# NTT123/vietTTS

Hardware: NVIDIA H100
Metric: audio_samples_per_sec (higher is better)
Workload: dtype f32 (bf16x3 split products on wgmma tensor cores, fp32 accumulate/storage)

## Files before the change

### viettts_b200/csrc/tc_conv.cu

```cuda
#include <cuda_bf16.h>

#include <algorithm>

#include "tc_common.cuh"
#include "vtts_internal.cuh"

namespace {

using namespace tcx;

constexpr int NCWG = 2;
constexpr int NCONS = NCWG * 128;
constexpr int PROD_WARP = NCONS / 32;
constexpr int NCONV = 96;
constexpr int NTHREADS = NCONS + 32 + NCONV;
constexpr int NA = 4;
constexpr int HALO = 64;
constexpr int PAIR_OVERLAP = 16;
constexpr int NQ = 2;
constexpr int NREADERS = (NCONS + NCONV) / 32;

constexpr int SUB_CG = 4;
constexpr int SUB_HALO = 1;
constexpr int SUB_RS = NCWG * 64 + SUB_HALO;
constexpr int SUB_CSB = SUB_RS * 64 + 32;
constexpr int SUB_STAGE = SUB_CG * SUB_CSB;
static_assert(SUB_RS * 4 % 32 == 4 && SUB_CSB / 4 % 32 == 24, "bank-conflict-free converter stores");

template <int N, int MW, int PAIRF, bool STAGED = false, bool SUB = false>
struct TcCfg {
  static constexpr int R = 64 * MW * NCWG;
  static constexpr int R_OUT = R - PAIR_OVERLAP;
  static constexpr int RA = R + HALO;
  static constexpr int A_STAGE = RA * 64;
  static constexpr int NAS = SUB ? (N == 64 ? 4 : 2) : NA;
  static constexpr int A_BYTES = SUB ? NAS * SUB_STAGE : NA * A_STAGE;
  static constexpr int W_STAGE = N * 64;
  static constexpr int NW = N == 256 ? 4 : 8;
  static constexpr int NCH2 = PAIRF ? N / 16 : 0;
  static constexpr int EPI_NC = N < 128 ? N : 128;
  static constexpr int EPI_LD = EPI_NC + 8;
  static constexpr int EPI_WG = 64 * EPI_LD + N;
  static constexpr int EPI_STAGE = STAGED ? NCWG * EPI_WG * 4 : 0;
  static constexpr int SMEM_BYTES =
      A_BYTES + NW * W_STAGE + NCH2 * A_STAGE + EPI_STAGE + (2 * NA + 2 * NW + 2 * NQ) * 8 + NQ * 4 + 1024;
  static_assert(SMEM_BYTES <= 227 * 1024, "shared memory of one CTA");
};

struct Ring {
  uint32_t s = 0, p = 0;
  template <int NS>
  __device__ __forceinline__ void next() { if (++s == NS) { s = 0; p ^= 1; } }
};

struct Tile {
  int pi, b, tt;
};
__device__ __forceinline__ Tile decode_tile(int t, int nprob, int tiles_per_row) {
  Tile d;
  d.pi = t % nprob; t /= nprob;
  d.tt = t % tiles_per_row;
  d.b = t / tiles_per_row;
  return d;
}

__device__ __forceinline__ int take_ticket(int* sched, int ntiles) {
  const int t = (int)gridDim.x + atomicAdd(&sched[0], 1);
  if (t < ntiles) return t;
  __threadfence();
  if (atomicAdd(&sched[1], 1) == (int)gridDim.x - 1) {
    atomicExch(&sched[0], 0);
    atomicExch(&sched[1], 0);
  }
  return -1;
}

struct TileQueue {
  int* id;
  uint64_t* full;
  uint64_t* empty;
  Ring r;
  __device__ __forceinline__ void put(int t, int* err, long long& acc) {
    mbar_wait_t(&empty[r.s], r.p ^ 1, err, 6, acc);
    id[r.s] = t;
    mbar_arrive(&full[r.s]);
    r.next<NQ>();
  }
  __device__ __forceinline__ int get(int* err, long long& acc) {
    int t = 0;
    if ((threadIdx.x & 31) == 0) {
      mbar_wait_t(&full[r.s], r.p, err, 6, acc);
      t = id[r.s];
      mbar_arrive(&empty[r.s]);
    }
    r.next<NQ>();
    return __shfl_sync(0xffffffffu, t, 0);
  }
};

__device__ __forceinline__ float div3_rn(float s) {
  constexpr float y = 0x1.555556p-2f;
  const float q0 = __fmul_rn(s, y);
  const float q1 = __fmaf_rn(__fmaf_rn(-q0, 3.0f, s), y, q0);
  return (s == 0.f || fabsf(s) == __int_as_float(0x7f800000)) ? s : q1;
}

template <int QN, int RS, int CSB, bool F16, bool LOADS_FIRST = false>
__device__ __forceinline__ void convert_rows(uint8_t* stage, int ct, const float* x0, const float* x1, const float* x2, int ld, int ch0,
                                             int row_base, int rows, int lo, int valid, int pre_mode, float slope) {
  static_assert(NCONV % QN == 0, "whole rows per converter step");
  constexpr int RSTEP = NCONV / QN, RA = RS;
  const int q = ct % QN;
  const int r0 = ct / QN;
  uint8_t* st = stage + (q >> 2) * CSB + (((q >> 1) & 1) * RA) * 16 + (q & 1) * 8;
  const int coff = ch0 + q * 4;
  constexpr int U = 8;
  for (int rr0 = r0; rr0 < rows; rr0 += RSTEP * U) {
    float4 v[U];
    if constexpr (LOADS_FIRST) {
      float4 a[U], bb[U];
      bool in[U];
#pragma unroll
      for (int u = 0; u < U; ++u) {
        const int rr = rr0 + u * RSTEP;
        const int t = row_base + rr;
        in[u] = rr < rows && t >= lo && t < valid;
        v[u] = a[u] = bb[u] = make_float4(0.f, 0.f, 0.f, 0.f);
        if (in[u]) {
          const size_t off = (size_t)t * ld + coff;
          v[u] = ldg_pf256(x0 + off);
          if (pre_mode == 2) {
            a[u] = ldg_pf256(x1 + off);
            bb[u] = ldg_pf256(x2 + off);
          }
        }
      }
#pragma unroll
      for (int u = 0; u < U; ++u) {
        if (in[u] && pre_mode == 2) {
          v[u].x = div3_rn((v[u].x + a[u].x) + bb[u].x);
          v[u].y = div3_rn((v[u].y + a[u].y) + bb[u].y);
          v[u].z = div3_rn((v[u].z + a[u].z) + bb[u].z);
          v[u].w = div3_rn((v[u].w + a[u].w) + bb[u].w);
        }
      }
    } else {
#pragma unroll
      for (int u = 0; u < U; ++u) {
        const int rr = rr0 + u * RSTEP;
        const int t = row_base + rr;
        v[u] = make_float4(0.f, 0.f, 0.f, 0.f);
        if (rr < rows && t >= lo && t < valid) {
          const size_t off = (size_t)t * ld + coff;
          v[u] = ldg_pf256(x0 + off);
          if (pre_mode == 2) {
            const float4 a = ldg_pf256(x1 + off);
            const float4 bb = ldg_pf256(x2 + off);
            v[u].x = ((v[u].x + a.x) + bb.x) / 3.0f;
            v[u].y = ((v[u].y + a.y) + bb.y) / 3.0f;
            v[u].z = ((v[u].z + a.z) + bb.z) / 3.0f;
            v[u].w = ((v[u].w + a.w) + bb.w) / 3.0f;
          }
        }
      }
    }
#pragma unroll
    for (int u = 0; u < U; ++u) {
      const int rr = rr0 + u * RSTEP;
      if (rr < rows) {
        float4 x = v[u];
        if (pre_mode >= 1) {
          x.x = lrelu(x.x, slope); x.y = lrelu(x.y, slope); x.z = lrelu(x.z, slope); x.w = lrelu(x.w, slope);
        }
        if constexpr (F16) {
          *reinterpret_cast<uint2*>(st + (size_t)rr * 16) = f16x4_sat(x);
        } else {
          uint2 hi, lo;
          split4(x, hi, lo);
          *reinterpret_cast<uint2*>(st + (size_t)rr * 16) = hi;
          *reinterpret_cast<uint2*>(st + (size_t)(2 * RA + rr) * 16) = lo;
        }
      }
    }
  }
}

template <int RA, bool F16>
__device__ __forceinline__ void convert_chunk(uint8_t* stage, int ct, const float* x0, const float* x1, const float* x2, int ld, int c,
                                              int row_base, int rows, int lo, int valid, int pre_mode, float slope) {
  convert_rows<4, RA, 0, F16>(stage, ct, x0, x1, x2, ld, c * 16, row_base, rows, lo, valid, pre_mode, slope);
}

template <int N, int NW, bool F16>
__device__ __forceinline__ void produce_weights(uint8_t* w_st, uint64_t* w_full, uint64_t* w_empty, Ring& rw, const void* wpk, int nch,
                                                int k, int* err, long long& wait_acc) {
  constexpr int WB = F16 ? N * 32 : N * 64;
  const uint8_t* src = reinterpret_cast<const uint8_t*>(wpk);
  for (int i = 0; i < nch * k; ++i) {
    mbar_wait_t(&w_empty[rw.s], rw.p ^ 1, err, 4, wait_acc);
// ... 247 lines not shown
            convert_rows<SUB_CG * 4, SUB_RS, SUB_CSB, F16, true>(a_st + ra.s * SUB_STAGE, ct, P.x0 + in_base, x1, x2, L.in_ld, c0 * 16,
                                                            tau0 + P.in_off + mt * NCWG * 64, NCWG * 64 + (k - 1) * dil, in_lo, valid,
                                                            L.pre_mode, L.pre_slope);
            fence_proxy_async();
            mbar_arrive(&a_full[ra.s]);
            ra.next<NAS>();
          }
      } else {
        for (int c = 0; c < nch; ++c) {
          mbar_wait_t(&a_empty[ra.s], ra.p ^ 1, L.err, 5, w_ae);
          convert_chunk<RA, F16>(a_st + ra.s * Cfg::A_STAGE, ct, P.x0 + in_base, x1, x2, L.in_ld, c, tau0 + P.in_off, R + (k - 1) * dil,
                            in_lo, valid, L.pre_mode, L.pre_slope);
          fence_proxy_async();
          mbar_arrive(&a_full[ra.s]);
          ra.next<NA>();
        }
      }
      (void)out_hi; (void)e_lim;
    TILE_LOOP_END
    if (L.dbg && ct == 0) L.dbg[(size_t)blockIdx.x * 16 + 5] = w_ae;
  } else {
    const int wg = warp >> 2, lane = tid & 31;
    float acc[MW][N / 2];
    Ring ra, rw;
    long long w_a = 0, w_w = 0, t_epi = 0;
    const long long t_begin = clock64();
    const int n_valid = (EPI && L.n_valid > 0) ? L.n_valid : N;
    const int post_act = EPI ? L.post_act : 0;
    constexpr int EPI_NC = Cfg::EPI_NC, EPI_LD = Cfg::EPI_LD, RPS = 128 / (EPI_NC / 4), NQ4 = 64 / RPS;
    float* stg = epi_st + wg * Cfg::EPI_WG;
    float* stg_bias = stg + 64 * EPI_LD;
    const int fr = (warp & 3) * 16 + (lane >> 2), fc = 2 * (lane & 3);
    const int dr = (tid & 127) / (EPI_NC / 4), dq = (tid & 127) % (EPI_NC / 4);
    READER_TILES
    TILE_LOOP_BEGIN
      const size_t out_base = (size_t)b * L.rows_out * (SUB ? L.out_sub : L.out_ld);
      const int ostride = P.out_stride, ooff = P.out_off, oe0 = SUB ? P.out_e0 : 0;
      auto row_ok = [&](int tau) { return (ROW_BOUNDS && P.rb) ? tau * ostride + ooff < out_hi : tau < valid; };
      auto elem_ok = [&](int tau, int e) { return SUB ? e >= 0 && e < e_lim : row_ok(tau); };
      auto blk_row = [&](int mt) { return tau0 + (SUB ? mt * NCWG + wg : wg * MW + mt) * 64; };
      auto fetch_pass = [&](int mt, int nh) {
        if (P.resid) {
          const int blk = blk_row(mt);
#pragma unroll
          for (int i = 0; i < NQ4; ++i) {
            const int row = i * RPS + dr, tau = blk + row;
            const int e = (tau * ostride + ooff) * L.out_ld + oe0 + nh * EPI_NC + dq * 4;
            if (elem_ok(tau, e)) cp_async16(stg + row * EPI_LD + dq * 4, P.resid + out_base + e);
          }
        }
        cp_async_commit();
      };
      auto wait_pass = [&]() {
        cp_async_wait_all();
        named_bar(2 + wg, 128);
      };
      if constexpr (EPI == 0) {
        if ((tid & 127) < N / 4) cp_async16(stg_bias + (tid & 127) * 4, P.bias + (tid & 127) * 4);
        fetch_pass(0, 0);
      }
      if constexpr (SUB) {
#pragma unroll
        for (int mt = 0; mt < MW; ++mt)
          consume_rows<N, NW, NAS, F16>(acc[mt], wg, smem_u32(a_st), a_full, a_empty, ra, smem_u32(w_st), w_full, w_empty, rw, nch, P.k,
                                        P.dil, L.err, w_a, w_w);
      } else {
        consume<N, MW, RA, NW, true, false, F16>(acc, wg, smem_u32(a_st), a_full, a_empty, ra, smem_u32(w_st), w_full, w_empty, rw, nch,
                                                 P.k, P.dil, L.err, w_a, w_w);
      }
      const long long t_epi0 = clock64();
      if constexpr (EPI == 0) {
        wait_pass();
#pragma unroll
        for (int mt = 0; mt < MW; ++mt) {
          const int blk = blk_row(mt);
          if (SUB ? sub_elem(L, P, blk, 0) >= e_lim : !row_ok(blk)) break;
#pragma unroll
          for (int nh = 0; nh < N / EPI_NC; ++nh) {
            if (mt + nh > 0 && P.resid) {
              fetch_pass(mt, nh);
              wait_pass();
            }
#pragma unroll
            for (int jn = 0; jn < EPI_NC / 8; ++jn) {
              const int col = jn * 8 + fc, e = (nh * (EPI_NC / 8) + jn) * 4;
              const float2 bi = *reinterpret_cast<const float2*>(stg_bias + nh * EPI_NC + col);
#pragma unroll
              for (int h = 0; h < 2; ++h) {
                float2* s = reinterpret_cast<float2*>(stg + (fr + 8 * h) * EPI_LD + col);
                float2 o = make_float2(acc[mt][e + 2 * h] + bi.x, acc[mt][e + 2 * h + 1] + bi.y);
                if (P.resid) {
                  const float2 r = *s;
                  o.x += r.x; o.y += r.y;
                }
                *s = o;
              }
            }
            named_bar(2 + wg, 128);
#pragma unroll
            for (int i = 0; i < NQ4; ++i) {
              const int row = i * RPS + dr, tau = blk + row;
              const int e = (tau * ostride + ooff) * L.out_ld + oe0 + nh * EPI_NC + dq * 4;
              if (elem_ok(tau, e))
                *reinterpret_cast<float4*>(P.out + out_base + e) = *reinterpret_cast<const float4*>(stg + row * EPI_LD + dq * 4);
            }
            named_bar(2 + wg, 128);
          }
        }
      } else {
        const int row_w = tau0 + wg * MW * 64 + (warp & 3) * 16 + (lane >> 2);
#pragma unroll
        for (int mt = 0; mt < MW; ++mt)
#pragma unroll
          for (int h = 0; h < 2; ++h) {
            const int tau = row_w + mt * 64 + 8 * h;
            if (!row_ok(tau)) continue;
            const size_t orow = out_base + (size_t)(tau * ostride + ooff) * L.out_ld;
#pragma unroll
            for (int jn = 0; jn < N / 8; ++jn) {
              const int col = jn * 8 + 2 * (lane & 3);
              if (col >= n_valid) continue;
              float2 o = make_float2(acc[mt][jn * 4 + 2 * h], acc[mt][jn * 4 + 2 * h + 1]);
              const float2 bi = __ldg(reinterpret_cast<const float2*>(P.bias + col));
              o.x += bi.x; o.y += bi.y;
              if (P.bn_mean) {
                const float2 mu = __ldg(reinterpret_cast<const float2*>(P.bn_mean + col));
                const float2 iv = __ldg(reinterpret_cast<const float2*>(P.bn_inv + col));
                const float2 of = __ldg(reinterpret_cast<const float2*>(P.bn_off + col));
                o.x = (o.x - mu.x) * iv.x + of.x; o.y = (o.y - mu.y) * iv.y + of.y;
              }
              if (post_act == 1) { o.x = tanhf(o.x); o.y = tanhf(o.y); }
              else if (post_act == 2) { o.x = fmaxf(o.x, 0.f); o.y = fmaxf(o.y, 0.f); }
              if (P.resid) {
                const float2 r = __ldg(reinterpret_cast<const float2*>(P.resid + orow + col));
                o.x += r.x; o.y += r.y;
              }
              *reinterpret_cast<float2*>(P.out + orow + col) = o;
            }
          }
      }
      t_epi += clock64() - t_epi0;
    TILE_LOOP_END
    if (L.dbg && tid == 0) {
      long long* d = L.dbg + (size_t)blockIdx.x * 16;
      d[0] = clock64() - t_begin; d[1] = t_epi; d[2] = w_a; d[3] = w_w;
    }
  }
#undef TILE_LOOP_BEGIN
#undef TILE_LOOP_END
}

template <int N, int MW, bool A2_REGS, bool F16>
__global__ void __launch_bounds__(NTHREADS, 1) tc_pair_kernel(const __grid_constant__ TcPairLaunch L) {
  using Cfg = TcCfg<N, MW, 1>;
  constexpr int R = Cfg::R, R_OUT = Cfg::R_OUT, RA = Cfg::RA, NW = Cfg::NW, NCH = N / 16;
  extern __shared__ uint8_t smem_raw[];
  uint8_t* smem = (uint8_t*)(((uintptr_t)smem_raw + 1023) & ~(uintptr_t)1023);
  uint8_t* a_st = smem;
  uint8_t* w_st = smem + NA * Cfg::A_STAGE;
  uint8_t* mid = w_st + NW * Cfg::W_STAGE;
  uint64_t* bars = reinterpret_cast<uint64_t*>(mid + Cfg::NCH2 * Cfg::A_STAGE);
  uint64_t* a_full = bars;
  uint64_t* a_empty = bars + NA;
  uint64_t* w_full = bars + 2 * NA;
  uint64_t* w_empty = bars + 2 * NA + NW;

  const int tid = threadIdx.x;
  const int warp = __shfl_sync(0xffffffffu, tid >> 5, 0);
  if (tid == 0) init_barriers(bars, NW);
  __syncthreads();

#define TILE_LOOP_BEGIN                                                   \
  for (int tile; (tile = next_tile()) >= 0;) {                            \
    const Tile td = decode_tile(tile, L.nprob, L.tiles_per_row);        \
    const int b = td.b;                                                    \
    const int tau0 = td.tt * R_OUT;                                        \
    int valid = L.T_rows;                                                 \
    if (L.len) {                                                          \
      const int v = L.len[b] * L.len_mul;                                 \
      valid = v < valid ? v : valid;                                      \
    }                                                                     \
    if (tau0 >= valid) continue;                                          \
    const TcPairProb& P = L.p[td.pi];                                      \
    const int k = P.k, dil = P.dil, h2 = (k - 1) / 2;
#define TILE_LOOP_END }

  if (warp == PROD_WARP) {
    if ((tid & 31) == 0) {
      Ring rw;
      long long w_e = 0;
      PRODUCER_TILES
      TILE_LOOP_BEGIN
        (void)b; (void)tau0; (void)dil; (void)h2;
        produce_weights<N, NW, F16>(w_st, w_full, w_empty, rw, P.w1pk, NCH, k, L.err, w_e);
        produce_weights<N, NW, F16>(w_st, w_full, w_empty, rw, P.w2pk, NCH, k, L.err, w_e);
      TILE_LOOP_END
    }
  } else if (warp > PROD_WARP) {
    const int ct = tid - NCONS - 32;
    Ring ra;
    long long w_ae = 0;
    READER_TILES
    TILE_LOOP_BEGIN
      const float* x = P.x + (size_t)b * L.T_rows * N;
      const int row_base = tau0 - h2 - (k - 1) * dil / 2;
      for (int c = 0; c < NCH; ++c) {
        mbar_wait_t(&a_empty[ra.s], ra.p ^ 1, L.err, 5, w_ae);
        convert_chunk<RA, F16>(a_st + ra.s * Cfg::A_STAGE, ct, x, nullptr, nullptr, N, c, row_base, R + (k - 1) * dil, 0, valid, 1, L.slope);
        fence_proxy_async();
        mbar_arrive(&a_full[ra.s]);
        ra.next<NA>();
      }
    TILE_LOOP_END
  } else {
    const int wg = warp >> 2, lane = tid & 31;
    float acc[MW][N / 2];
    Ring ra, rw;
    long long w_a = 0, w_w = 0;
    const long long t_begin = clock64();
    const float slope = L.slope;
    READER_TILES
    TILE_LOOP_BEGIN
      consume<N, MW, RA, NW, true, false, F16>(acc, wg, smem_u32(a_st), a_full, a_empty, ra, smem_u32(w_st), w_full, w_empty, rw, NCH, k, dil,
                                               L.err, w_a, w_w);
      const int lr_w = wg * MW * 64 + (warp & 3) * 16 + (lane >> 2);
#pragma unroll
      for (int mt = 0; mt < MW; ++mt)
#pragma unroll
        for (int h = 0; h < 2; ++h) {
          const int lr = lr_w + mt * 64 + 8 * h;
          const int u = tau0 - h2 + lr;
          const bool inside = u >= 0 && u < valid;
#pragma unroll
          for (int jn = 0; jn < N / 8; ++jn) {
            const int col = jn * 8 + 2 * (lane & 3);
            const float2 bi = __ldg(reinterpret_cast<const float2*>(P.b1 + col));
            const float v0 = inside ? lrelu(acc[mt][jn * 4 + 2 * h] + bi.x, slope) : 0.f;
            const float v1 = inside ? lrelu(acc[mt][jn * 4 + 2 * h + 1] + bi.y, slope) : 0.f;
            uint8_t* dst = mid + (col >> 4) * Cfg::A_STAGE + (((col >> 3) & 1) * RA + lr) * 16 + (col & 7) * 2;
            if constexpr (F16) {
              *reinterpret_cast<uint32_t*>(dst) = f16x2_sat(v0, v1);
            } else {
              const __nv_bfloat162 hi = __floats2bfloat162_rn(v0, v1);
              const __nv_bfloat162 lo = __floats2bfloat162_rn(v0 - __low2float(hi), v1 - __high2float(hi));
              *reinterpret_cast<__nv_bfloat162*>(dst) = hi;
              *reinterpret_cast<__nv_bfloat162*>(dst + 2 * RA * 16) = lo;
            }
          }
        }
      fence_proxy_async();
      named_bar(1, NCONS);
      consume<N, MW, RA, NW, false, A2_REGS, F16>(acc, wg, smem_u32(mid), a_full, a_empty, ra, smem_u32(w_st), w_full, w_empty, rw, NCH, k, 1,
                                                  L.err, w_a, w_w);
      named_bar(1, NCONS);
      const float* x = P.x + (size_t)b * L.T_rows * N;
      float* out = P.out + (size_t)b * L.T_rows * N;
#pragma unroll
      for (int mt = 0; mt < MW; ++mt)
#pragma unroll
        for (int h = 0; h < 2; ++h) {
          const int lr = lr_w + mt * 64 + 8 * h;
          const int tau = tau0 + lr;
          if (lr >= R_OUT || tau >= valid) continue;
#pragma unroll
          for (int jn = 0; jn < N / 8; ++jn) {
            const int col = jn * 8 + 2 * (lane & 3);
            const float2 bi = __ldg(reinterpret_cast<const float2*>(P.b2 + col));
            const float2 r = __ldg(reinterpret_cast<const float2*>(x + (size_t)tau * N + col));
            float2 o;
            o.x = acc[mt][jn * 4 + 2 * h] + bi.x + r.x;
            o.y = acc[mt][jn * 4 + 2 * h + 1] + bi.y + r.y;
            *reinterpret_cast<float2*>(out + (size_t)tau * N + col) = o;
          }
        }
    TILE_LOOP_END
    if (L.dbg && tid == 0) {
      long long* d = L.dbg + (size_t)blockIdx.x * 16;
      d[0] = clock64() - t_begin; d[2] = w_a; d[3] = w_w;
    }
  }
#undef TILE_LOOP_BEGIN
#undef TILE_LOOP_END
}

template <bool F16>
__global__ void pack_w_kernel(const float* __restrict__ w, uint16_t* __restrict__ dst, int k, int Cin, int Cout_total, int n0, int N) {
  const size_t total = (size_t)k * Cin * N;
  for (size_t idx = blockIdx.x * (size_t)blockDim.x + threadIdx.x; idx < total; idx += (size_t)gridDim.x * blockDim.x) {
    const int n = idx % N;
    const int i = (idx / N) % Cin;
    const int j = idx / ((size_t)N * Cin);
    const float v = (n0 + n) < Cout_total ? w[((size_t)j * Cin + i) * Cout_total + n0 + n] : 0.f;
    const int c = i / 16, kh = (i % 16) / 8, e = i % 8;
    if constexpr (F16) {
      const size_t blk = ((size_t)c * k + j) * (size_t)(2 * N * 8);
      dst[blk + ((size_t)kh * N + n) * 8 + e] = (uint16_t)(f16x2_sat(v, 0.f) & 0xffffu);
      continue;
    }
    const __nv_bfloat16 hi = __float2bfloat16_rn(v);
    const __nv_bfloat16 lo = __float2bfloat16_rn(v - __bfloat162float(hi));
    const size_t blk = ((size_t)c * k + j) * (size_t)(4 * N * 8);
    dst[blk + ((size_t)(kh * 2 + 0) * N + n) * 8 + e] = __bfloat16_as_ushort(hi);
    dst[blk + ((size_t)(kh * 2 + 1) * N + n) * 8 + e] = __bfloat16_as_ushort(lo);
  }
}

template <int N, int EPI, int MW, bool F16, bool SUB = false>
int launch_cfg(vtts_ctx* ctx, TcLaunch& L, cudaStream_t st) {
  using Cfg = TcCfg<N, MW, 0, EPI == 0, SUB>;
  static bool attr_done_dev[64] = {};
  if (!attr_done_dev[ctx->device & 63]) {
    VTTS_CUDA(cudaFuncSetAttribute(tc_conv_kernel<N, EPI, MW, F16, SUB>, cudaFuncAttributeMaxDynamicSharedMemorySize, Cfg::SMEM_BYTES));
    attr_done_dev[ctx->device & 63] = true;
  }
  for (int i = 0; i < L.nprob; ++i)
    if ((L.p[i].k - 1) * L.p[i].dil > (SUB ? SUB_HALO : HALO)) return ctx->fail(VTTS_ERR_BAD_ARG, "tc_conv: halo too large");
  if (SUB && L.Cin % (SUB_CG * 16)) return ctx->fail(VTTS_ERR_BAD_ARG, "tc_conv: sub-row output needs Cin %% %d == 0, not %d", SUB_CG * 16, L.Cin);
  std::stable_sort(L.p, L.p + L.nprob, [](const TcProb& a, const TcProb& b) { return a.k > b.k; });
  L.tiles_per_row = ((L.tile_rows > 0 ? L.tile_rows : L.T_rows) + Cfg::R - 1) / Cfg::R;
  L.ntiles = L.nprob * L.tiles_per_row * L.B;
  const int grid = L.ntiles < ctx->sm_count ? L.ntiles : ctx->sm_count;
  tc_conv_kernel<N, EPI, MW, F16, SUB><<<grid, NTHREADS, Cfg::SMEM_BYTES, st>>>(L);
  ctx->launches++;
  VTTS_CUDA(cudaGetLastError());
  return VTTS_OK;
}

template <int N>
int launch_n(vtts_ctx* ctx, TcLaunch& L, cudaStream_t st) {
  constexpr int MW = N >= 256 ? 1 : (N == 128 ? 2 : 4);
  bool generic = L.post_act != 0 || (L.n_valid > 0 && L.n_valid < N);
  bool rb = false;
  for (int i = 0; i < L.nprob; ++i) {
    generic |= L.p[i].bn_mean != nullptr;
    rb |= L.p[i].rb != nullptr;
  }
  if ((rb || L.out_sub) && generic) return ctx->fail(VTTS_ERR_BAD_ARG, "tc_conv: per-row bounds and sub-row output use the plain epilogue");
  if (L.out_sub < 0 || (L.out_sub && (L.out_sub % 4 || L.out_ld % L.out_sub)))
    return ctx->fail(VTTS_ERR_BAD_ARG, "tc_conv: output rows of %d floats in tile rows of %d", L.out_sub, L.out_ld);
  if (!generic) {
    const int row_w = L.out_sub ? L.out_sub : L.out_ld;
    if ((int64_t)L.rows_out * row_w > INT32_MAX) return ctx->fail(VTTS_ERR_BAD_ARG, "tc_conv: %d output rows of %d", L.rows_out, row_w);
    bool aligned = L.out_ld % 4 == 0;
    for (int i = 0; i < L.nprob; ++i) aligned &= (((uintptr_t)L.p[i].out | (uintptr_t)L.p[i].resid | (uintptr_t)L.p[i].bias) & 15) == 0;
    if (!aligned) return ctx->fail(VTTS_ERR_BAD_ARG, "tc_conv: the plain epilogue needs 16-byte aligned out / resid rows and bias (out_ld %d)", L.out_ld);
  }
  if (L.f16 && generic) return ctx->fail(VTTS_ERR_BAD_ARG, "tc_conv: fp16 operands use the plain epilogue");
  if (L.f16) return L.out_sub ? launch_cfg<N, 0, MW, true, true>(ctx, L, st) : launch_cfg<N, 0, MW, true>(ctx, L, st);
  if (generic) return launch_cfg<N, 1, MW, false>(ctx, L, st);
  return L.out_sub ? launch_cfg<N, 0, MW, false, true>(ctx, L, st) : launch_cfg<N, 0, MW, false>(ctx, L, st);
}

template <int N, int MW, bool A2_REGS, bool F16 = false>
int launch_pair(vtts_ctx* ctx, TcPairLaunch& L, cudaStream_t st) {
  using Cfg = TcCfg<N, MW, 1>;
  static bool attr_done_dev[64] = {};
  if (!attr_done_dev[ctx->device & 63]) {
    VTTS_CUDA(cudaFuncSetAttribute(tc_pair_kernel<N, MW, A2_REGS, F16>, cudaFuncAttributeMaxDynamicSharedMemorySize, Cfg::SMEM_BYTES));
    attr_done_dev[ctx->device & 63] = true;
  }
  for (int i = 0; i < L.nprob; ++i)
    if (L.p[i].k - 1 > PAIR_OVERLAP || (L.p[i].k - 1) * L.p[i].dil > HALO) return ctx->fail(VTTS_ERR_BAD_ARG, "tc_pair: halo too large");
  std::stable_sort(L.p, L.p + L.nprob, [](const TcPairProb& a, const TcPairProb& b) { return a.k > b.k; });
  L.tiles_per_row = (L.T_rows + Cfg::R_OUT - 1) / Cfg::R_OUT;
  L.ntiles = L.nprob * L.tiles_per_row * L.B;
  const int grid = L.ntiles < ctx->sm_count ? L.ntiles : ctx->sm_count;
  tc_pair_kernel<N, MW, A2_REGS, F16><<<grid, NTHREADS, Cfg::SMEM_BYTES, st>>>(L);
  ctx->launches++;
  VTTS_CUDA(cudaGetLastError());
  return VTTS_OK;
}

}

size_t vtts_tc_packed_elems(int k, int Cin, int N, bool f16) { return (size_t)k * Cin * N * (f16 ? 1 : 2); }

int vtts_tc_pack_weights(vtts_ctx* ctx, const float* w, void* dst, int k, int Cin, int Cout_total, int n0, int N, bool f16) {
  if (f16) pack_w_kernel<true><<<256, 256>>>(w, reinterpret_cast<uint16_t*>(dst), k, Cin, Cout_total, n0, N);
  else pack_w_kernel<false><<<256, 256>>>(w, reinterpret_cast<uint16_t*>(dst), k, Cin, Cout_total, n0, N);
  VTTS_CUDA(cudaGetLastError());
  return VTTS_OK;
}

int vtts_tc_tile_n(int Cout) { return Cout <= 32 ? 32 : (Cout <= 64 ? 64 : (Cout <= 128 ? 128 : 256)); }

size_t vtts_tc_conv_packed_bytes(int k, int Cin, int Cout, bool f16) {
  const int N = vtts_tc_tile_n(Cout), nt = (Cout + N - 1) / N;
  return ((vtts_tc_packed_elems(k, Cin, N, f16) * 2 + 255) & ~size_t(255)) * nt;
}

int vtts_tc_pack_conv(vtts_ctx* ctx, const float* w, int k, int Cin, int Cout, bool f16, char*& cursor, std::vector<void*>& out) {
  const int N = vtts_tc_tile_n(Cout), nt = (Cout + N - 1) / N;
  for (int t = 0; t < nt; ++t) {
    int rc = vtts_tc_pack_weights(ctx, w, cursor, k, Cin, Cout, t * N, N, f16);
    if (rc) return rc;
    out.push_back(cursor);
    cursor += (vtts_tc_packed_elems(k, Cin, N, f16) * 2 + 255) & ~size_t(255);
  }
  return VTTS_OK;
}

int vtts_conv_dispatch(vtts_ctx* ctx, const ConvLaunch& L, void* const* wpk, cudaStream_t st) {
  if (ctx->precision == VTTS_PRECISION_FP32 || wpk == nullptr) return vtts_launch_conv(ctx, L, st);
  const int N = vtts_tc_tile_n(L.Cout), nt = (L.Cout + N - 1) / N;
  TcLaunch TL;
  auto reset = [&]() {
    memset(&TL, 0, sizeof(TL));
    TL.Cin = L.Cin; TL.N = N; TL.in_ld = L.Cin; TL.out_ld = L.Cout; TL.B = L.B; TL.T_rows = L.T_rows; TL.rows_out = L.rows_out;
    TL.len = L.len; TL.len_mul = L.len_mul; TL.pre_mode = L.pre_mode; TL.pre_slope = L.pre_slope; TL.post_act = L.post_act;
    TL.n_valid = (L.Cout % N) ? (L.Cout % N) : N;
  };
  reset();
  for (int pass = 0; pass < 2; ++pass) {
    const bool partial = pass == 1;
    if (partial && (L.Cout % N) == 0) break;
    reset();
    TL.n_valid = partial ? (L.Cout % N) : N;
    for (int pi = 0; pi < L.nprob; ++pi) {
      const ConvProb& cp = L.p[pi];
      for (int t = 0; t < nt; ++t) {
        const bool is_partial = (t == nt - 1) && (L.Cout % N) != 0;
        if (is_partial != partial) continue;
        const int n0 = t * N;
        TcProb q;
        memset(&q, 0, sizeof(q));
        q.x0 = cp.x0; q.x1 = cp.x1; q.x2 = cp.x2;
        q.wpk = wpk[pi * nt + t];
        q.bias = cp.bias + n0;
        q.resid = cp.resid ? cp.resid + n0 : nullptr;
        if (cp.bn_mean) { q.bn_mean = cp.bn_mean + n0; q.bn_inv = cp.bn_inv + n0; q.bn_off = cp.bn_off + n0; }
        q.out = cp.out + n0;
        q.k = cp.k; q.dil = cp.dil; q.in_off = cp.in_off; q.out_stride = cp.out_stride; q.out_off = cp.out_off;
        TL.p[TL.nprob++] = q;
        if (TL.nprob == 8) {
          int rc = vtts_launch_tc_conv(ctx, TL, st);
          if (rc) return rc;
          TL.nprob = 0;
        }
      }
    }
    if (TL.nprob > 0) {
      int rc = vtts_launch_tc_conv(ctx, TL, st);
      if (rc) return rc;
    }
  }
  return VTTS_OK;
}

int vtts_launch_tc_conv(vtts_ctx* ctx, TcLaunch& L, cudaStream_t st) {
  if (L.nprob < 1 || L.nprob > 8) return ctx->fail(VTTS_ERR_BAD_ARG, "tc_conv: nprob %d", L.nprob);
  if (L.Cin % 16 != 0) return ctx->fail(VTTS_ERR_BAD_ARG, "tc_conv: Cin %d", L.Cin);
  for (int i = 0; i < L.nprob; ++i)
    if (L.p[i].k < 1) return ctx->fail(VTTS_ERR_BAD_ARG, "tc_conv: k");
  L.sched = ctx->d_tc_sched;
  L.err = ctx->d_err;
  L.dbg = ctx->tc_dbg_on ? ctx->d_tc_dbg : nullptr;
  switch (L.N) {
    case 256: return launch_n<256>(ctx, L, st);
    case 128: return launch_n<128>(ctx, L, st);
    case 64: return launch_n<64>(ctx, L, st);
    case 32: return launch_n<32>(ctx, L, st);
    default: return ctx->fail(VTTS_ERR_BAD_ARG, "tc_conv: N %d unsupported", L.N);
  }
}

int vtts_launch_tc_pair(vtts_ctx* ctx, TcPairLaunch& L, cudaStream_t st) {
  if (L.nprob < 1 || L.nprob > 3) return ctx->fail(VTTS_ERR_BAD_ARG, "tc_pair: nprob %d", L.nprob);
  for (int i = 0; i < L.nprob; ++i)
    if (L.p[i].k < 1 || L.p[i].x == L.p[i].out) return ctx->fail(VTTS_ERR_BAD_ARG, "tc_pair: bad problem %d", i);
  L.sched = ctx->d_tc_sched;
  L.err = ctx->d_err;
  L.dbg = ctx->tc_dbg_on ? ctx->d_tc_dbg : nullptr;
  if (L.N != 32 && L.N != 64) return ctx->fail(VTTS_ERR_BAD_ARG, "tc_pair: C %d unsupported (32 or 64)", L.N);
  if (L.f16) {
    if (ctx->pair_ts != 2) return ctx->fail(VTTS_ERR_BAD_ARG, "tc_pair: fp16 operands exist for the default pair form (256-row tiles) only, not form %d", ctx->pair_ts);
    return L.N == 64 ? launch_pair<64, 2, false, true>(ctx, L, st) : launch_pair<32, 2, false, true>(ctx, L, st);
  }
  if (ctx->pair_ts == 1) return L.N == 64 ? launch_pair<64, 2, true>(ctx, L, st) : launch_pair<32, 2, true>(ctx, L, st);
  if (ctx->pair_ts == 0) return L.N == 64 ? launch_pair<64, 1, false>(ctx, L, st) : launch_pair<32, 1, false>(ctx, L, st);
  return L.N == 64 ? launch_pair<64, 2, false>(ctx, L, st) : launch_pair<32, 2, false>(ctx, L, st);
}
```

### viettts_b200/engine.py

```python
from __future__ import annotations

import ctypes as C
import threading
from typing import NamedTuple

import numpy as np

from . import _lib, config, weights

DROPOUT_OFF, DROPOUT_MASK, DROPOUT_SEED, DROPOUT_REFERENCE = 0, 1, 2, 3


def _chunk_seed(seed: int, chunk: int) -> int:
    return (int(seed) ^ (chunk * 0x9E3779B97F4A7C15)) & 0xFFFFFFFFFFFFFFFF


def _rng_seed(rng, *others) -> int:
    if any(o is not None for o in others):
        raise ValueError("rng= selects the reference's own mask stream; it cannot be combined with masks= or seed=")
    w = np.asarray(rng).ravel()
    if w.size != 2 or not np.issubdtype(w.dtype, np.integer):
        raise ValueError(f"rng must hold exactly two integer words (the checkpoint's uint32[2] rng), got {np.asarray(rng).shape}")
    return ((int(w[0]) & 0xFFFFFFFF) << 32) | (int(w[1]) & 0xFFFFFFFF)
PRECISION_FP32, PRECISION_BF16X3, PRECISION_FP16 = 0, 1, 2
# ... 155 lines not shown

def _keyed_params(what: str, spec, ranges: dict, presets: dict) -> dict:
    if isinstance(spec, str):
        given = {}
        s = spec.strip().lower()
        if s not in presets:
            for item in s.split(","):
                key, eq, val = item.strip().partition("=")
                if not eq:
                    raise ValueError(f"{what}: {item.strip()!r} is not key=value (keys {', '.join(ranges)}) "
                                     f"or a preset ({', '.join(presets)})")
                given[key.strip()] = val.strip()
    elif isinstance(spec, dict):
        given = dict(spec)
    else:
        raise ValueError(f"{what}: a spec is a string or a dict, got {type(spec).__name__}")
    out = dict(presets["voice"])
    for key, val in given.items():
        if key not in ranges:
            raise ValueError(f"{what}: unknown key {key!r} (keys {', '.join(ranges)})")
        try:
            v = float(np.float32(float(val)))
        except (TypeError, ValueError):
            raise ValueError(f"{what}: {key}={val!r} is not a number") from None
        lo, hi = ranges[key]
        if not (np.isfinite(v) and lo <= v <= hi):
            raise ValueError(f"{what}: {key}={val} must lie in [{lo:g}, {hi:g}]")
        out[key] = v
    for key, v in out.items():
        lo, hi = ranges[key]
        if not lo <= v <= hi:
            raise ValueError(f"{what}: {key}={v:g} (the voice preset's) must lie in [{lo:g}, {hi:g}] at this rate")
    return out


def _ptr(a):
    if a is None:
        return None
    if isinstance(a, np.ndarray):
        return a.ctypes.data
    return a.data_ptr()


def _np(a, dtype, shape=None, what="array"):
    a = np.ascontiguousarray(np.asarray(a), dtype=dtype)
    if shape is not None and tuple(a.shape) != tuple(shape):
        raise ValueError(f"{what}: expected shape {tuple(shape)}, got {tuple(a.shape)}")
    return a


def _wav_rows(wav, lengths=None):
    x = _np(wav, np.float32)
    one = x.ndim == 1
    x = x[None] if one else x
    if x.ndim != 2:
        raise ValueError(f"wav must be [S] or [B,S], got {np.shape(wav)}")
    return x, None if lengths is None else _np(lengths, np.int32, (x.shape[0],), "lengths"), one


def _out_tensor(out, shape, device, what="out"):
    import torch
    if out is None:
        return torch.empty(shape, dtype=torch.float32, device=device)
    if tuple(out.shape) != shape or out.dtype != torch.float32 or not out.is_contiguous() or out.device != torch.device(device):
        raise ValueError(f"{what} must be contiguous float32 [{', '.join(map(str, shape))}] on {device}")
    return out


def _dev_rows(x_t, out, stream, width=None):
    import torch
    assert x_t.is_cuda and x_t.dtype == torch.float32 and x_t.is_contiguous() and x_t.dim() == 2
    B, S = x_t.shape
    out = _out_tensor(out, (B, S if width is None else width), x_t.device)
    return B, S, out, torch.cuda.current_stream(x_t.device).cuda_stream if stream is None else stream


class Engine:

    def __init__(self, device: int = 0):
        self.lib = _lib.load()
        self.device = int(device)
        h = _lib.c_ctx()
        rc = self.lib.vtts_create(self.device, C.byref(h))
        if rc != 0:
            msg = self.lib.vtts_last_error(None)
            raise _lib.VttsError(rc, msg.decode() if msg else "?")
        self.h = h
        self._hifigan_key = None
        self._acoustic_key = None
        self._duration_key = None
        self._mel_fb = None
        self._denoise_bias = None

    def close(self):
        if getattr(self, "h", None):
            self.lib.vtts_destroy(self.h)
            self.h = None

    def __del__(self):
        try:
            self.close()
        except Exception:
            pass

    def _ck(self, rc):
        _lib.check(self.h, rc)

    def device_info(self) -> dict:
        sm, ma, mi, hb = C.c_int(), C.c_int(), C.c_int(), C.c_int64()
        self._ck(self.lib.vtts_device_info(self.h, C.byref(sm), C.byref(ma), C.byref(mi), C.byref(hb)))
        return dict(sm_count=sm.value, cc=(ma.value, mi.value), hbm_bytes=hb.value)

    def launch_count(self) -> int:
        return int(self.lib.vtts_launch_count(self.h))

    def last_stage_ms(self, stage: int) -> float:
        ms = C.c_float()
        self._ck(self.lib.vtts_last_stage_ms(self.h, stage, C.byref(ms)))
        return float(ms.value)

    def set_precision(self, mode) -> None:
        m = PRECISIONS.get(mode, mode)
        self._ck(self.lib.vtts_set_precision(self.h, int(m)))
        self._denoise_bias = None

    def debug_conv1d(self, precision, x_t, w_t, bias_t, k, dil, pre_slope=1.0, resid_t=None, len_t=None):
        import torch
        B, T, Cin = x_t.shape
        Cout = w_t.shape[2]
        out = torch.empty((B, T, Cout), dtype=torch.float32, device=x_t.device)
        m = PRECISIONS.get(precision, precision)
        self._ck(self.lib.vtts_debug_conv1d(self.h, int(m), _ptr(x_t), _ptr(w_t), _ptr(bias_t), _ptr(resid_t), _ptr(len_t),
                                            B, T, Cin, Cout, int(k), int(dil), float(pre_slope), _ptr(out)))
        return out

    POST_ACTS = {"none": 0, "tanh": 1, "relu": 2}

    def debug_conv_dispatch(self, precision, xs, ws, biases, k, dil=1, bns=None, resids=None, post_act="none", len_t=None, outs=None):
        import torch
        n = len(xs)
        B, T, Cin = xs[0].shape
        Cout = ws[0].shape[2]
        if outs is None:
            outs = [torch.empty((B, T, Cout), dtype=torch.float32, device=xs[0].device) for _ in range(n)]

        def arr(ts):
            return None if ts is None else (C.c_void_p * n)(*[_ptr(t) for t in ts])

        m = PRECISIONS.get(precision, precision)
        self._ck(self.lib.vtts_debug_conv_dispatch(self.h, int(m), n, arr(xs), arr(ws), arr(biases), arr(bns), arr(resids), arr(outs),
                                                   _ptr(len_t), B, T, Cin, Cout, int(k), int(dil), self.POST_ACTS[post_act]))
        return outs

    def debug_pair(self, x_t, w1_t, b1_t, w2_t, b2_t, k, dil, slope=0.1, len_t=None):
        import torch
        B, T, Cc = x_t.shape
        out = torch.empty_like(x_t)
        self._ck(self.lib.vtts_debug_pair(self.h, _ptr(x_t), _ptr(w1_t), _ptr(b1_t), _ptr(w2_t), _ptr(b2_t), _ptr(len_t),
                                          B, T, Cc, int(k), int(dil), float(slope), _ptr(out)))
        return out

    HIFIGAN_LAYERS = 18

    def debug_hifigan_layer(self, layer, xs, outs, n_frames_t=None, T=None):
        scale = [1, 1, 8, 64, 128] + [8] * 3 + [64] * 3 + [128] * 3 + [256] * 3 + [256]
        B, rows = xs[0].shape[:2]
        if T is None:
            T = rows // scale[layer]
        arr = lambda ts: (C.c_void_p * len(ts))(*[_ptr(t) for t in ts])
        self._ck(self.lib.vtts_debug_hifigan_layer(self.h, int(layer), arr(xs), arr(outs), _ptr(n_frames_t), int(B), int(T)))
        return outs

    PAIR_KERNELS = {"smem": 0, "tmem": 1, "smem2": 2}

    def set_fused_pairs(self, on: bool, kind: str | None = None):
        flags = 0x200 | ((1 if on else 0) << 10)
        if kind is not None:
            flags |= 0x800 | (self.PAIR_KERNELS[kind] << 12)
        self._ck(self.lib.vtts_debug_tc_stats(self.h, flags, None))
        self._denoise_bias = None

    def tc_stats(self, enable=True):
        out = np.zeros((256, 16), np.int64)
        self._ck(self.lib.vtts_debug_tc_stats(self.h, 1 if enable else 0, _ptr(out)))
        return out

    SUBSTAGES = {1: "acoustic.encoder", 2: "acoustic.upsample", 3: "acoustic.cond_gemm", 4: "acoustic.decoder_scan",
                 5: "acoustic.projection", 6: "acoustic.postnet", 9: "hifigan.conv_pre", 10: "hifigan.stage0", 11: "hifigan.stage1",
                 12: "hifigan.stage2", 13: "hifigan.stage3", 14: "hifigan.conv_post", 17: "teacher.encoder_upsample",
                 18: "teacher.prenet_hoisted_gemm", 19: "teacher.zoneout_scan", 20: "teacher.projection_postnet"}

    def substages(self, enable=True) -> dict:
        out = np.zeros(24, np.float32)
        self._ck(self.lib.vtts_debug_substages(self.h, 1 if enable else 0, _ptr(out)))
        return {name: float(out[i]) for i, name in self.SUBSTAGES.items() if out[i] > 0}

    def _load(self, fn, pack, src):
        blob = pack(src) if isinstance(src, dict) else src
        n = int(blob.size if isinstance(blob, np.ndarray) else blob.numel())
        if isinstance(blob, np.ndarray):
            blob = _np(blob, np.float32)
        self._ck(fn(self.h, _ptr(blob), n))

    def load_hifigan(self, params, key=None):
        self._load(self.lib.vtts_load_hifigan, weights.pack_hifigan, params)
        self._hifigan_key = key if key is not None else object()
        self._denoise_bias = None

    def load_acoustic(self, ckpt, key=None):
        self._load(self.lib.vtts_load_acoustic, weights.pack_acoustic, ckpt)
        self._acoustic_key = key if key is not None else object()

    def load_duration(self, ckpt, key=None):
        self._load(self.lib.vtts_load_duration, weights.pack_duration, ckpt)
        self._duration_key = key if key is not None else object()

    def broadcast_weights(self, nccl_comm, root: int, is_root: bool, stream=None):
        self._ck(self.lib.vtts_broadcast_weights(self.h, nccl_comm, int(root), 1 if is_root else 0, stream))
        self._denoise_bias = None
        if not is_root:
            self._hifigan_key = self._acoustic_key = self._duration_key = object()

    def load_mel_filterbank(self, fb=None):
        fb = _np(weights.mel_filterbank() if fb is None else fb, np.float32, (config.MEL_DIM, config.N_FFT // 2 + 1), "filterbank").copy()
        self._mel_fb = None
        self._ck(self.lib.vtts_load_mel_filterbank(self.h, _ptr(fb), fb.shape[0], fb.shape[1]))
        self._mel_fb = fb

    def mel2wave(self, mel, n_frames=None, out=None) -> np.ndarray:
        mel = _np(mel, np.float32)
        if mel.ndim != 3 or mel.shape[2] != config.MEL_DIM:
            raise ValueError(f"mel must be [B,T,{config.MEL_DIM}], got {mel.shape}")
        B, T, _ = mel.shape
        nf = None if n_frames is None else _np(n_frames, np.int32, (B,), "n_frames")
        if out is not None and (out.shape != (B, T * config.HOP) or out.dtype != np.float32 or not out.flags.c_contiguous):
            raise ValueError(f"out must be C-contiguous float32 {(B, T * config.HOP)}")
        wav = out if out is not None else np.empty((B, T * config.HOP), np.float32)
        self._ck(self.lib.vtts_mel2wave_host(self.h, _ptr(mel), _ptr(nf), B, T, _ptr(wav)))
        return wav

    STREAM_HALO = 16

    def mel2wave_stream(self, mel, chunk_frames: int = 32, halo: int | None = None):
        mel = _np(mel, np.float32)
        if mel.ndim == 3:
            if mel.shape[0] != 1:
                raise ValueError("mel2wave_stream takes one utterance ([T,80] or [1,T,80])")
            mel = mel[0]
        if mel.ndim != 2 or mel.shape[1] != config.MEL_DIM:
            raise ValueError(f"mel must be [T,{config.MEL_DIM}], got {mel.shape}")
        halo = self.STREAM_HALO if halo is None else int(halo)
        if chunk_frames < 1 or halo < 0:
            raise ValueError("chunk_frames >= 1 and halo >= 0 required")
        T = mel.shape[0]
        for t0 in range(0, T, chunk_frames):
            t1 = min(T, t0 + chunk_frames)
            a, b = max(0, t0 - halo), min(T, t1 + halo)
            wav = self.mel2wave(mel[None, a:b])[0]
            yield wav[(t0 - a) * config.HOP: (t1 - a) * config.HOP]

    def open_vocoder_stream(self, max_streams: int, max_chunk_frames: int) -> "VocoderStream":
        return VocoderStream(self, max_streams, max_chunk_frames)

    def open_acoustic_stream(self, max_streams: int, max_chunk_frames: int, max_frames: int, max_tokens: int, seed=None, rng=None,
                             masks: bool = False) -> "AcousticStream":
        return AcousticStream(self, max_streams, max_chunk_frames, max_frames, max_tokens, seed=seed, rng=rng, masks=masks)

    def open_tts_stream(self, max_streams: int, max_chunk_frames: int, max_frames: int, max_tokens: int = 1024, seed=None,
                        rng=None, output_rate=None, denoise=None, meter=False, semitones=None, tempo=None, limit=None,
                        gain_db=0.0, eq=None, compress=None, deess=None) -> "TtsStream":
        return TtsStream(self, max_streams, max_chunk_frames, max_frames, max_tokens, seed=seed, rng=rng, output_rate=output_rate,
                         denoise=denoise, meter=meter, semitones=semitones, tempo=tempo, limit=limit, gain_db=gain_db, eq=eq,
                         compress=compress, deess=deess)

    def tts_plan(self, tokens, lengths=None, silence_duration=-1.0):
        tokens = _np(tokens, np.int32)
        if tokens.ndim != 2:
            raise ValueError("tokens must be [B,L]")
        B, L = tokens.shape
        lens = None if lengths is None else _np(lengths, np.int32, (B,), "lengths")
        sec = np.empty((B, L), np.float32)
        frames = np.empty((B, L), np.float32)
        nf = np.empty(B, np.int32)
        ne = np.empty(B, np.int32)
        self._ck(self.lib.vtts_tts_plan(self.h, _ptr(tokens), _ptr(lens), B, L, float(silence_duration), _ptr(sec), _ptr(frames),
                                        _ptr(nf), _ptr(ne)))
        return sec, frames, nf, ne

    def get_precision(self) -> int:
        return int(self.lib.vtts_get_precision(self.h))

    def _acoustic_args(self, tokens, dur_frames, lengths, n_frames, masks, seed, rng=None):
        ref_seed = None if rng is None else _rng_seed(rng, masks, seed)
        tokens = _np(tokens, np.int32)
        if tokens.ndim != 2:
            raise ValueError("tokens must be [B,L]")
        B, L = tokens.shape
        dur = _np(dur_frames, np.float32, (B, L), "durations")
        lens = None if lengths is None else _np(lengths, np.int32, (B,), "lengths")
        if n_frames is None:
            from .nat.text2mel import frame_count
            nf = np.array([frame_count(dur[b, : (L if lens is None else lens[b])]) for b in range(B)], np.int32)
        else:
            nf = _np(n_frames, np.int32, (B,), "n_frames")
        N = int(nf.max())
        if N < 1:
            raise ValueError("durations sum to less than one frame")
        if ref_seed is not None:
            return tokens, dur, lens, nf, N, None, DROPOUT_REFERENCE, ref_seed
        if masks is not None:
# ... 1206 lines not shown
```

Before: 58.11 million.

## Stage pair-kernel residual epilogue through shared memory with cp.async prefetch

The fused conv pair kernel now prefetches the residual input rows and both bias vectors into a per-warpgroup shared staging buffer with cp.async while conv1 runs. The epilogue adds bias and residual in shared memory and writes out coalesced float4 rows, replacing scattered float2 global loads and stores from the MMA fragment layout. The intermediate buffer gets its own row stride (RM) sized for the pair overlap. This uses more shared memory and adds named barriers and extra passes when the staging buffer cannot hold all row blocks.

Result: no change. 58.25 million (median of 6 runs) (+0.2%).

```diff
diff --git a/viettts_b200/csrc/tc_conv.cu b/viettts_b200/csrc/tc_conv.cu
--- a/viettts_b200/csrc/tc_conv.cu
+++ b/viettts_b200/csrc/tc_conv.cu
@@ -38,13 +38,22 @@
   static constexpr int W_STAGE = N * 64;
   static constexpr int NW = N == 256 ? 4 : 8;
   static constexpr int NCH2 = PAIRF ? N / 16 : 0;
+  static constexpr int RM = R + PAIR_OVERLAP;
+  static constexpr int M_STAGE = RM * 64;
   static constexpr int EPI_NC = N < 128 ? N : 128;
   static constexpr int EPI_LD = EPI_NC + 8;
-  static constexpr int EPI_WG = 64 * EPI_LD + N;
+  static constexpr int EPI_OFF = A_BYTES + NW * W_STAGE + NCH2 * M_STAGE;
+  static constexpr int BARS_BYTES = (2 * NA + 2 * NW + 2 * NQ) * 8 + NQ * 4 + 1024;
+  static constexpr int EPI_NB =
+      PAIRF && EPI_OFF + NCWG * (64 * MW * EPI_LD + 2 * N) * 4 + BARS_BYTES <= 227 * 1024 ? MW : 1;
+  static constexpr int EPI_WG = 64 * EPI_NB * EPI_LD + (PAIRF ? 2 : 1) * N;
   static constexpr int EPI_STAGE = STAGED ? NCWG * EPI_WG * 4 : 0;
-  static constexpr int SMEM_BYTES =
-      A_BYTES + NW * W_STAGE + NCH2 * A_STAGE + EPI_STAGE + (2 * NA + 2 * NW + 2 * NQ) * 8 + NQ * 4 + 1024;
+  static constexpr int SMEM_BYTES = EPI_OFF + EPI_STAGE + BARS_BYTES;
   static_assert(SMEM_BYTES <= 227 * 1024, "shared memory of one CTA");
+  static_assert(EPI_LD % 32 == 8 && EPI_OFF % 16 == 0 && EPI_WG % 4 == 0, "bank-conflict-free, 16-byte aligned staging rows");
+  static_assert(!PAIRF || (STAGED && N == EPI_NC && MW % EPI_NB == 0 && R - 1 + PAIR_OVERLAP < RM && R_OUT - 1 + PAIR_OVERLAP < R),
+                "pair kernel: one staging pass per EPI_NB 64-row blocks; every row conv2 reads lies in the intermediate, "
+                "and the stored rows read only rows conv1 wrote");
 };
 
 struct Ring {
@@ -598,14 +607,15 @@
 
 template <int N, int MW, bool A2_REGS, bool F16>
 __global__ void __launch_bounds__(NTHREADS, 1) tc_pair_kernel(const __grid_constant__ TcPairLaunch L) {
-  using Cfg = TcCfg<N, MW, 1>;
-  constexpr int R = Cfg::R, R_OUT = Cfg::R_OUT, RA = Cfg::RA, NW = Cfg::NW, NCH = N / 16;
+  using Cfg = TcCfg<N, MW, 1, true>;
+  constexpr int R = Cfg::R, R_OUT = Cfg::R_OUT, RA = Cfg::RA, RM = Cfg::RM, NW = Cfg::NW, NCH = N / 16;
   extern __shared__ uint8_t smem_raw[];
   uint8_t* smem = (uint8_t*)(((uintptr_t)smem_raw + 1023) & ~(uintptr_t)1023);
   uint8_t* a_st = smem;
   uint8_t* w_st = smem + NA * Cfg::A_STAGE;
   uint8_t* mid = w_st + NW * Cfg::W_STAGE;
-  uint64_t* bars = reinterpret_cast<uint64_t*>(mid + Cfg::NCH2 * Cfg::A_STAGE);
+  float* epi_st = reinterpret_cast<float*>(smem_raw + (smem + Cfg::EPI_OFF - smem_raw));
+  uint64_t* bars = reinterpret_cast<uint64_t*>(smem + Cfg::EPI_OFF + Cfg::EPI_STAGE);
   uint64_t* a_full = bars;
   uint64_t* a_empty = bars + NA;
   uint64_t* w_full = bars + 2 * NA;
@@ -662,67 +672,119 @@
     const int wg = warp >> 2, lane = tid & 31;
     float acc[MW][N / 2];
     Ring ra, rw;
-    long long w_a = 0, w_w = 0;
+    long long w_a = 0, w_w = 0, t_epi = 0, t_mid = 0;
     const long long t_begin = clock64();
     const float slope = L.slope;
+    constexpr int EPI_LD = Cfg::EPI_LD, NB = Cfg::EPI_NB, RPS = 128 / (N / 4), NQ4 = 64 / RPS;
+    float* stg = epi_st + wg * Cfg::EPI_WG;
+    float* stg_b2 = stg + 64 * NB * EPI_LD;
+    float* stg_b1 = stg_b2 + N;
+    const int fr = (warp & 3) * 16 + (lane >> 2), fc = 2 * (lane & 3);
+    const int dr = (tid & 127) / (N / 4), dq = (tid & 127) % (N / 4);
     READER_TILES
     TILE_LOOP_BEGIN
+      const float* x = P.x + (size_t)b * L.T_rows * N;
+      float* out = P.out + (size_t)b * L.T_rows * N;
+      auto row_ok = [&](int lr) { return lr < R_OUT && tau0 + lr < valid; };
+      auto fetch_pass = [&](int p) {
+#pragma unroll
+        for (int nb = 0; nb < NB; ++nb) {
+          const int lr0 = (wg * MW + p * NB + nb) * 64;
+#pragma unroll
+          for (int i = 0; i < NQ4; ++i) {
+            const int row = nb * 64 + i * RPS + dr, lr = lr0 + i * RPS + dr;
+            if (row_ok(lr)) cp_async16(stg + row * EPI_LD + dq * 4, x + (size_t)(tau0 + lr) * N + dq * 4);
+          }
+        }
+        cp_async_commit();
+      };
+      auto wait_pass = [&]() {
+        cp_async_wait_all();
+        named_bar(2 + wg, 128);
+      };
+      if ((tid & 127) < N / 4) {
+        cp_async16(stg_b2 + (tid & 127) * 4, P.b2 + (tid & 127) * 4);
+        cp_async16(stg_b1 + (tid & 127) * 4, P.b1 + (tid & 127) * 4);
+      }
+      fetch_pass(0);
       consume<N, MW, RA, NW, true, false, F16>(acc, wg, smem_u32(a_st), a_full, a_empty, ra, smem_u32(w_st), w_full, w_empty, rw, NCH, k, dil,
                                                L.err, w_a, w_w);
-      const int lr_w = wg * MW * 64 + (warp & 3) * 16 + (lane >> 2);
+      const long long t_mid0 = clock64();
+      wait_pass();
 #pragma unroll
       for (int mt = 0; mt < MW; ++mt)
 #pragma unroll
         for (int h = 0; h < 2; ++h) {
-          const int lr = lr_w + mt * 64 + 8 * h;
+          const int lr = (wg * MW + mt) * 64 + fr + 8 * h;
           const int u = tau0 - h2 + lr;
           const bool inside = u >= 0 && u < valid;
 #pragma unroll
           for (int jn = 0; jn < N / 8; ++jn) {
-            const int col = jn * 8 + 2 * (lane & 3);
-            const float2 bi = __ldg(reinterpret_cast<const float2*>(P.b1 + col));
+            const int col = jn * 8 + fc;
+            const float2 bi = *reinterpret_cast<const float2*>(stg_b1 + col);
             const float v0 = inside ? lrelu(acc[mt][jn * 4 + 2 * h] + bi.x, slope) : 0.f;
             const float v1 = inside ? lrelu(acc[mt][jn * 4 + 2 * h + 1] + bi.y, slope) : 0.f;
-            uint8_t* dst = mid + (col >> 4) * Cfg::A_STAGE + (((col >> 3) & 1) * RA + lr) * 16 + (col & 7) * 2;
+            uint8_t* dst = mid + (col >> 4) * Cfg::M_STAGE + (((col >> 3) & 1) * RM + lr) * 16 + (col & 7) * 2;
             if constexpr (F16) {
               *reinterpret_cast<uint32_t*>(dst) = f16x2_sat(v0, v1);
             } else {
               const __nv_bfloat162 hi = __floats2bfloat162_rn(v0, v1);
               const __nv_bfloat162 lo = __floats2bfloat162_rn(v0 - __low2float(hi), v1 - __high2float(hi));
               *reinterpret_cast<__nv_bfloat162*>(dst) = hi;
-              *reinterpret_cast<__nv_bfloat162*>(dst + 2 * RA * 16) = lo;
+              *reinterpret_cast<__nv_bfloat162*>(dst + 2 * RM * 16) = lo;
             }
           }
         }
       fence_proxy_async();
       named_bar(1, NCONS);
-      consume<N, MW, RA, NW, false, A2_REGS, F16>(acc, wg, smem_u32(mid), a_full, a_empty, ra, smem_u32(w_st), w_full, w_empty, rw, NCH, k, 1,
+      t_mid += clock64() - t_mid0;
+      consume<N, MW, RM, NW, false, A2_REGS, F16>(acc, wg, smem_u32(mid), a_full, a_empty, ra, smem_u32(w_st), w_full, w_empty, rw, NCH, k, 1,
                                                   L.err, w_a, w_w);
+      const long long t_epi0 = clock64();
       named_bar(1, NCONS);
-      const float* x = P.x + (size_t)b * L.T_rows * N;
-      float* out = P.out + (size_t)b * L.T_rows * N;
-#pragma unroll
-      for (int mt = 0; mt < MW; ++mt)
-#pragma unroll
-        for (int h = 0; h < 2; ++h) {
-          const int lr = lr_w + mt * 64 + 8 * h;
-          const int tau = tau0 + lr;
-          if (lr >= R_OUT || tau >= valid) continue;
+#pragma unroll
+      for (int p = 0; p < MW / NB; ++p) {
+        if (!row_ok((wg * MW + p * NB) * 64)) break;
+        if (p > 0) {
+          fetch_pass(p);
+          wait_pass();
+        }
+#pragma unroll
+        for (int nb = 0; nb < NB; ++nb) {
+          const int mt = p * NB + nb;
 #pragma unroll
           for (int jn = 0; jn < N / 8; ++jn) {
-            const int col = jn * 8 + 2 * (lane & 3);
-            const float2 bi = __ldg(reinterpret_cast<const float2*>(P.b2 + col));
-            const float2 r = __ldg(reinterpret_cast<const float2*>(x + (size_t)tau * N + col));
-            float2 o;
-            o.x = acc[mt][jn * 4 + 2 * h] + bi.x + r.x;
-            o.y = acc[mt][jn * 4 + 2 * h + 1] + bi.y + r.y;
-            *reinterpret_cast<float2*>(out + (size_t)tau * N + col) = o;
+            const int col = jn * 8 + fc;
+            const float2 bi = *reinterpret_cast<const float2*>(stg_b2 + col);
+#pragma unroll
+            for (int h = 0; h < 2; ++h) {
+              float2* st = reinterpret_cast<float2*>(stg + (nb * 64 + fr + 8 * h) * EPI_LD + col);
+              const float2 r = *st;
+              float2 o;
+              o.x = acc[mt][jn * 4 + 2 * h] + bi.x + r.x;
+              o.y = acc[mt][jn * 4 + 2 * h + 1] + bi.y + r.y;
+              *st = o;
+            }
           }
         }
+        named_bar(2 + wg, 128);
+#pragma unroll
+        for (int nb = 0; nb < NB; ++nb) {
+          const int lr0 = (wg * MW + p * NB + nb) * 64;
+#pragma unroll
+          for (int i = 0; i < NQ4; ++i) {
+            const int row = nb * 64 + i * RPS + dr, lr = lr0 + i * RPS + dr;
+            if (row_ok(lr))
+              *reinterpret_cast<float4*>(out + (size_t)(tau0 + lr) * N + dq * 4) = *reinterpret_cast<const float4*>(stg + row * EPI_LD + dq * 4);
+          }
+        }
+        named_bar(2 + wg, 128);
+      }
+      t_epi += clock64() - t_epi0;
     TILE_LOOP_END
     if (L.dbg && tid == 0) {
       long long* d = L.dbg + (size_t)blockIdx.x * 16;
-      d[0] = clock64() - t_begin; d[2] = w_a; d[3] = w_w;
+      d[0] = clock64() - t_begin; d[1] = t_epi; d[2] = w_a; d[3] = w_w; d[9] = t_mid;
     }
   }
 #undef TILE_LOOP_BEGIN
@@ -799,14 +861,18 @@
 
 template <int N, int MW, bool A2_REGS, bool F16 = false>
 int launch_pair(vtts_ctx* ctx, TcPairLaunch& L, cudaStream_t st) {
-  using Cfg = TcCfg<N, MW, 1>;
+  using Cfg = TcCfg<N, MW, 1, true>;
   static bool attr_done_dev[64] = {};
   if (!attr_done_dev[ctx->device & 63]) {
     VTTS_CUDA(cudaFuncSetAttribute(tc_pair_kernel<N, MW, A2_REGS, F16>, cudaFuncAttributeMaxDynamicSharedMemorySize, Cfg::SMEM_BYTES));
     attr_done_dev[ctx->device & 63] = true;
   }
-  for (int i = 0; i < L.nprob; ++i)
-    if (L.p[i].k - 1 > PAIR_OVERLAP || (L.p[i].k - 1) * L.p[i].dil > HALO) return ctx->fail(VTTS_ERR_BAD_ARG, "tc_pair: halo too large");
+  for (int i = 0; i < L.nprob; ++i) {
+    const TcPairProb& p = L.p[i];
+    if (p.k - 1 > PAIR_OVERLAP || (p.k - 1) * p.dil > HALO) return ctx->fail(VTTS_ERR_BAD_ARG, "tc_pair: halo too large");
+    if ((((uintptr_t)p.x | (uintptr_t)p.out | (uintptr_t)p.b1 | (uintptr_t)p.b2) & 15) != 0)
+      return ctx->fail(VTTS_ERR_BAD_ARG, "tc_pair: x, out, b1 and b2 must be 16-byte aligned (problem %d)", i);
+  }
   std::stable_sort(L.p, L.p + L.nprob, [](const TcPairProb& a, const TcPairProb& b) { return a.k > b.k; });
   L.tiles_per_row = (L.T_rows + Cfg::R_OUT - 1) / Cfg::R_OUT;
   L.ntiles = L.nprob * L.tiles_per_row * L.B;
diff --git a/viettts_b200/engine.py b/viettts_b200/engine.py
--- a/viettts_b200/engine.py
+++ b/viettts_b200/engine.py
@@ -331,10 +331,11 @@
                                                    _ptr(len_t), B, T, Cin, Cout, int(k), int(dil), self.POST_ACTS[post_act]))
         return outs
 
-    def debug_pair(self, x_t, w1_t, b1_t, w2_t, b2_t, k, dil, slope=0.1, len_t=None):
+    def debug_pair(self, x_t, w1_t, b1_t, w2_t, b2_t, k, dil, slope=0.1, len_t=None, out=None):
         import torch
         B, T, Cc = x_t.shape
-        out = torch.empty_like(x_t)
+        if out is None:
+            out = torch.empty_like(x_t)
         self._ck(self.lib.vtts_debug_pair(self.h, _ptr(x_t), _ptr(w1_t), _ptr(b1_t), _ptr(w2_t), _ptr(b2_t), _ptr(len_t),
                                           B, T, Cc, int(k), int(dil), float(slope), _ptr(out)))
         return out
```
